# codelaboratoryltd/bng

Measured on AMD Instinct MI355X. Metric: mpps, higher is better.
Workload: dtype uint8; 1 GPU; model=bng-uplink-pipeline (dhcp_fastpath+antispoof+nat44+qos), benchmark=Mpps + p50 DHCP OFFER latency, 64B mix, 1M-sub table at 1/2/4/8 MI355X, global_batch=1048576, seq_len=512, svc_cus=0, parallelism=shard1-rss-dhcp-alltoall, n_subscribers=1000000

## Files before the change

bng_amd/dataplane/csrc/bng_device.h:

```cpp
#ifndef BNG_DEVICE_H
#define BNG_DEVICE_H

#include <hip/hip_runtime.h>
#include "bng_abi.h"

#define BNG_DEV __device__ __forceinline__

BNG_DEV uint64_t bng_mix64(uint64_t x) {
  x += 0x9E3779B97F4A7C15ULL;
  uint64_t z = x;
  z = (z ^ (z >> 30)) * 0xBF58476D1CE4E5B9ULL;
  z = (z ^ (z >> 27)) * 0x94D049BB133111EBULL;
  return z ^ (z >> 31);
}

BNG_DEV uint64_t bng_fnv1a64(const uint8_t* p, int n) {
  uint64_t h = 0xCBF29CE484222325ULL;
  for (int i = 0; i < n; ++i) { h ^= p[i]; h *= 0x100000001B3ULL; }
  return h;
}

BNG_DEV uint64_t bng_tuple_sig(uint32_t src_ip, uint32_t dst_ip,
                               uint16_t src_port, uint16_t dst_port,
                               uint8_t proto) {
  uint64_t a = ((uint64_t)src_ip << 32) | dst_ip;
  uint64_t b = ((uint64_t)src_port << 24) | ((uint64_t)dst_port << 8) | proto;
  uint64_t s = bng_mix64(bng_mix64(a) ^ b);
  s |= 1ULL;
  if (s == BNG_KEY_TOMBSTONE) s -= 2;
  return s;
}

BNG_DEV uint64_t bng_eim_sig(uint32_t ip, uint16_t port, uint8_t proto) {
  uint64_t s = bng_mix64(((uint64_t)ip << 24) | ((uint64_t)port << 8) | proto);
  s |= 1ULL;
  if (s == BNG_KEY_TOMBSTONE) s -= 2;
  return s;
}

BNG_DEV uint8_t  ld_u8 (const uint8_t* p)  { return *p; }
BNG_DEV uint16_t ld_u16be(const uint8_t* p) {
  return ((uint16_t)p[0] << 8) | p[1];
}
BNG_DEV uint32_t ld_u32be(const uint8_t* p) {
  return ((uint32_t)p[0] << 24) | ((uint32_t)p[1] << 16) |
         ((uint32_t)p[2] << 8) | p[3];
}
BNG_DEV void st_u16be(uint8_t* p, uint16_t v) {
  p[0] = (uint8_t)(v >> 8); p[1] = (uint8_t)v;
}
BNG_DEV void st_u32be(uint8_t* p, uint32_t v) {
  p[0] = (uint8_t)(v >> 24); p[1] = (uint8_t)(v >> 16);
  p[2] = (uint8_t)(v >> 8);  p[3] = (uint8_t)v;
}
BNG_DEV void bng_zero(uint8_t* p, int n) {
  int i = 0;
  while (((uintptr_t)(p + i) & 3) && i < n) p[i++] = 0;
  for (; i + 16 <= n && !((uintptr_t)(p + i) & 15); i += 16)
    *(uint4*)(p + i) = make_uint4(0, 0, 0, 0);
  for (; i + 4 <= n; i += 4) *(uint32_t*)(p + i) = 0;
  while (i < n) p[i++] = 0;
}

BNG_DEV void stat_inc(unsigned long long* counter, bool cond) {
  uint64_t mask = __ballot(cond);
  if (mask == 0) return;
  int leader = __ffsll((unsigned long long)mask) - 1;
  int lane = threadIdx.x & 63;
  if (lane == leader)
    atomicAdd(counter, (unsigned long long)__popcll(mask));
}

BNG_DEV uint32_t wave_count(bool cond) {
  return (uint32_t)__popcll((unsigned long long)__ballot(cond));
}

BNG_DEV uint32_t wave_sum32(uint32_t v) {
  for (int off = 32; off > 0; off >>= 1)
    v += __shfl_down(v, off, 64);
  return (uint32_t)__builtin_amdgcn_readfirstlane((int)v);
}

BNG_DEV void sb_zero(unsigned long long* sb, int n) {
  if ((int)threadIdx.x < n) sb[threadIdx.x] = 0;
  __syncthreads();
}

BNG_DEV void sb_fold(unsigned long long* sb, int slot, uint64_t cnt) {
  if (cnt && (threadIdx.x & 63) == 0)
    atomicAdd(&sb[slot], (unsigned long long)cnt);
}

BNG_DEV void sb_commit(const unsigned long long* sb, int base, int n,
                       unsigned long long* counters) {
  int k = (int)threadIdx.x - base;
  if (k >= 0 && k < n) {
    unsigned long long v = sb[base + k];
    if (v) atomicAdd(&counters[k], v);
  }
}

BNG_DEV void bng_publish_ready(uint8_t* ready_flag) {
  __builtin_amdgcn_fence(__ATOMIC_RELEASE, "agent");
  asm volatile("s_waitcnt vmcnt(0)" ::: "memory");
  __hip_atomic_store(ready_flag, (uint8_t)1, __ATOMIC_RELAXED,
                     __HIP_MEMORY_SCOPE_AGENT);
}

BNG_DEV bool bng_wait_ready(const uint8_t* ready_flag, int max_spins) {
  for (int i = 0; i < max_spins; ++i) {
    if (__hip_atomic_load(ready_flag, __ATOMIC_RELAXED,
                          __HIP_MEMORY_SCOPE_AGENT)) {
      __builtin_amdgcn_fence(__ATOMIC_ACQUIRE, "agent");
      return true;
    }
    __builtin_amdgcn_s_sleep(1);
  }
  return false;
}

BNG_DEV uint32_t ring_claim(bng_ring_header* hdr) {
  return atomicAdd(&hdr->widx, 1u);
}

#endif
```

bng_amd/dataplane/csrc/bng_kernels.hip:

```cpp
#include <hip/hip_runtime.h>
#include "bng_abi.h"
#include "bng_params.h"
#include "bng_device.h"
#include "bng_launch.h"


typedef __attribute__((address_space(1))) uint64_t gu64_t;

BNG_DEV uint64_t rlx_load64(const void* ptr) {
  return __hip_atomic_load((const uint64_t*)ptr, __ATOMIC_RELAXED,
                           __HIP_MEMORY_SCOPE_AGENT);
}
BNG_DEV void rlx_store64(void* ptr, uint64_t v) {
  __hip_atomic_store((uint64_t*)ptr, v, __ATOMIC_RELAXED,
                     __HIP_MEMORY_SCOPE_AGENT);
}

#ifndef BNG_SC1_PROBES
#define BNG_SC1_PROBES 1
#endif
BNG_DEV uint4 ld_probe16(const void* p) {
#if BNG_SC1_PROBES
  const uint64_t* q = (const uint64_t*)p;
  uint64_t a = rlx_load64(q), b = rlx_load64(q + 1);
// ... 113 lines not shown
  return &t[(slot + my_pos) & mask];
}

template <typename E>
BNG_DEV E* sig_find_or_claim(E* t, uint32_t mask, uint64_t sig,
                             bool* claimed, bool* found) {
  *claimed = false; *found = false;
  uint32_t slot = (uint32_t)sig & mask;
  for (int i = 0; i < BNG_MAX_PROBE; ++i) {
    E* e = &t[(slot + i) & mask];
    uint64_t k = __hip_atomic_load(&e->sig, __ATOMIC_RELAXED,
                                   __HIP_MEMORY_SCOPE_AGENT);
    if (k == sig) { *found = true; return e; }
    if (k == BNG_KEY_EMPTY) break;
  }
  for (int attempt = 0; attempt < 4; ++attempt) {
    int first_tomb = -1, first_tomb_pos = -1;
    for (int i = 0; i < BNG_MAX_PROBE; ++i) {
      E* e = &t[(slot + i) & mask];
      uint64_t k = __hip_atomic_load(&e->sig, __ATOMIC_RELAXED,
                                     __HIP_MEMORY_SCOPE_AGENT);
      if (k == sig) { *found = true; return e; }
      if (k == BNG_KEY_TOMBSTONE) {
        if (first_tomb < 0) {
          first_tomb = (int)((slot + i) & mask);
          first_tomb_pos = i;
        }
        continue;
      }
      if (k == BNG_KEY_EMPTY) {
        E* d = first_tomb >= 0 ? &t[first_tomb] : e;
        int d_pos = first_tomb >= 0 ? first_tomb_pos : i;
        uint64_t want = first_tomb >= 0 ? BNG_KEY_TOMBSTONE
                                        : BNG_KEY_EMPTY;
        if (__hip_atomic_compare_exchange_strong(
                &d->sig, &want, sig, __ATOMIC_RELAXED, __ATOMIC_RELAXED,
                __HIP_MEMORY_SCOPE_AGENT)) {
          return claim_dedup(t, mask, sig, slot, d_pos, claimed, found);
        }
        if (want == sig) { *found = true; return d; }
        if (first_tomb >= 0) { first_tomb = -1; first_tomb_pos = -1; --i; }
        continue;
      }
    }
    if (first_tomb < 0)
      return nullptr;
    E* d = &t[first_tomb];
    uint64_t want = BNG_KEY_TOMBSTONE;
    if (__hip_atomic_compare_exchange_strong(
            &d->sig, &want, sig, __ATOMIC_RELAXED, __ATOMIC_RELAXED,
            __HIP_MEMORY_SCOPE_AGENT)) {
      return claim_dedup(t, mask, sig, slot, first_tomb_pos, claimed,
                         found);
    }
    if (want == sig) { *found = true; return d; }
  }
  return nullptr;
}

template <typename E>
BNG_DEV E* sig_lookup(E* t, uint32_t mask, uint64_t sig) {
  uint32_t slot = (uint32_t)sig & mask;
  for (int i = 0; i < BNG_MAX_PROBE; ++i) {
    E* e = &t[(slot + i) & mask];
    uint64_t k = __hip_atomic_load(&e->sig, __ATOMIC_RELAXED,
                                   __HIP_MEMORY_SCOPE_AGENT);
    if (k == sig) return e;
    if (k == BNG_KEY_EMPTY) return nullptr;
  }
  return nullptr;
}

template <auto K, typename E>
BNG_DEV E* key_upsert_slot(E* t, uint32_t mask, uint64_t key) {
  uint32_t slot = (uint32_t)bng_mix64(key) & mask;
  E* tomb = nullptr;
  for (int i = 0; i < BNG_MAX_PROBE; ++i) {
    E* e = &t[(slot + i) & mask];
    uint64_t cur = rlx_load64(&(e->*K));
    if (cur == key) return e;
    if (cur == BNG_KEY_TOMBSTONE && !tomb) tomb = e;
    if (cur == BNG_KEY_EMPTY) {
      E* d = tomb ? tomb : e;
      uint64_t expect = tomb ? BNG_KEY_TOMBSTONE : BNG_KEY_EMPTY;
      if (__hip_atomic_compare_exchange_strong(
              &(d->*K), &expect, key, __ATOMIC_RELAXED, __ATOMIC_RELAXED,
              __HIP_MEMORY_SCOPE_AGENT))
        return d;
      tomb = nullptr;
    }
  }
  return nullptr;
}

template <auto K, typename E>
BNG_DEV E* key_find(E* t, uint32_t mask, uint64_t key) {
  uint32_t slot = (uint32_t)bng_mix64(key) & mask;
  for (int i = 0; i < BNG_MAX_PROBE; ++i) {
    E* e = &t[(slot + i) & mask];
    uint64_t cur = rlx_load64(&(e->*K));
    if (cur == key) return e;
    if (cur == BNG_KEY_EMPTY) return nullptr;
  }
  return nullptr;
}

template <typename E>
BNG_DEV E* ipkey_upsert_slot(E* t, uint32_t mask, uint32_t ip,
                             bool claim_if_absent, bool* full) {
  *full = false;
  uint32_t slot = (uint32_t)bng_mix64(ip) & mask;
  for (int i = 0; i < BNG_MAX_PROBE; ++i) {
    E* e = &t[(slot + i) & mask];
    uint32_t cur = __hip_atomic_load(&e->key_ip, __ATOMIC_RELAXED,
                                     __HIP_MEMORY_SCOPE_AGENT);
    if (cur == ip) return e;
    if (cur == 0) {
      if (!claim_if_absent) return nullptr;
      if (__hip_atomic_compare_exchange_strong(
              &e->key_ip, &cur, ip, __ATOMIC_RELAXED, __ATOMIC_RELAXED,
              __HIP_MEMORY_SCOPE_AGENT))
        return e;
    }
  }
  *full = true;
  return nullptr;
}

BNG_DEV bool tuple_eq(const bng_nat_tuple& a, const bng_nat_tuple& b) {
  return a.src_ip == b.src_ip && a.dst_ip == b.dst_ip &&
         a.src_port == b.src_port && a.dst_port == b.dst_port &&
         a.protocol == b.protocol;
}


struct pktctx {
  uint8_t* p;
  int len;
  int ip_off;
  int l4_off;
  uint8_t proto;
  uint32_t saddr, daddr;
  uint16_t sport, dport;
  uint16_t icmp_id;
  uint8_t tcp_flags;
  int vlan_offset;
  uint16_t s_tag, c_tag;
  bool tagged;
  bool l4_ok;
  uint32_t W[12];
  bool regs;
};

#define RG_B(c, o) (((c).W[(o) >> 2] >> (24 - 8 * ((o) & 3))) & 0xFFu)
BNG_DEV uint16_t rg_ld16(const pktctx& c, int o) {
  return (uint16_t)((RG_B(c, o) << 8) | RG_B(c, o + 1));
}
BNG_DEV void rg_st8(pktctx& c, int o, uint32_t v) {
  int i = o >> 2, sh = 24 - 8 * (o & 3);
  c.W[i] = (c.W[i] & ~(0xFFu << sh)) | ((v & 0xFFu) << sh);
}
BNG_DEV void rg_st16(pktctx& c, int o, uint32_t v) {
  rg_st8(c, o, v >> 8); rg_st8(c, o + 1, v);
}
BNG_DEV void rg_st32(pktctx& c, int o, uint32_t v) {
  rg_st16(c, o, v >> 16); rg_st16(c, o + 2, v);
}
BNG_DEV void rg_flush16_47(pktctx& c) {
  uint4* q = (uint4*)c.p;
  q[1] = make_uint4(__builtin_bswap32(c.W[4]), __builtin_bswap32(c.W[5]),
                    __builtin_bswap32(c.W[6]), __builtin_bswap32(c.W[7]));
  q[2] = make_uint4(__builtin_bswap32(c.W[8]), __builtin_bswap32(c.W[9]),
                    __builtin_bswap32(c.W[10]),
                    __builtin_bswap32(c.W[11]));
}

BNG_DEV bool parse_pkt_fast(pktctx& c, uint8_t* p, int len) {
  if (len < 48 || ((uintptr_t)p & 15)) return false;
  #pragma unroll
  for (int i = 0; i < 3; ++i) {
    uint4 v = ((const uint4*)p)[i];
    c.W[i * 4 + 0] = __builtin_bswap32(v.x);
    c.W[i * 4 + 1] = __builtin_bswap32(v.y);
    c.W[i * 4 + 2] = __builtin_bswap32(v.z);
    c.W[i * 4 + 3] = __builtin_bswap32(v.w);
  }
  #define BNG_B(o) ((c.W[(o) >> 2] >> (24 - 8 * ((o) & 3))) & 0xFFu)
  #define BNG_H(o) ((BNG_B(o) << 8) | BNG_B((o) + 1))
  uint32_t ethertype = BNG_H(12);
  if (ethertype != 0x0800) return false;
  if (BNG_B(14) != 0x45) return false;
  c.p = p; c.len = len; c.vlan_offset = 0; c.s_tag = c.c_tag = 0;
  c.tagged = false; c.l4_ok = false;
  c.regs = true;
  c.ip_off = 14;
  c.proto = (uint8_t)BNG_B(23);
  c.saddr = (BNG_H(26) << 16) | BNG_H(28);
  c.daddr = (BNG_H(30) << 16) | BNG_H(32);
  c.l4_off = 34;
  if (c.proto == 6 && len >= 54) {
    c.sport = (uint16_t)BNG_H(34);
    c.dport = (uint16_t)BNG_H(36);
    c.tcp_flags = (uint8_t)BNG_B(47);
    c.l4_ok = true;
  } else if (c.proto == 17 && len >= 42) {
    c.sport = (uint16_t)BNG_H(34);
    c.dport = (uint16_t)BNG_H(36);
    c.l4_ok = true;
  } else if (c.proto == 1 && len >= 42) {
    c.icmp_id = (uint16_t)BNG_H(38);
    c.l4_ok = true;
  }
  #undef BNG_B
  #undef BNG_H
  return true;
}

BNG_DEV bool parse_pkt_slow(pktctx& c, uint8_t* p, int len, bool want_vlan) {
  c.p = p; c.len = len; c.ip_off = -1; c.vlan_offset = 0;
  c.s_tag = c.c_tag = 0; c.tagged = false; c.l4_ok = false;
  c.regs = false;
  if (len < 14) return false;
  uint16_t proto = ld_u16be(p + 12);
  int off = 14;
  if (want_vlan && (proto == 0x8100 || proto == 0x88A8)) {
    if (len < off + 4) return false;
    c.tagged = true;
    c.s_tag = ld_u16be(p + off) & 0xFFF;
    proto = ld_u16be(p + off + 2);
    off += 4; c.vlan_offset = 4;
    if (proto == 0x8100) {
      if (len < off + 4) return false;
      c.c_tag = ld_u16be(p + off) & 0xFFF;
      proto = ld_u16be(p + off + 2);
      off += 4; c.vlan_offset = 8;
    }
  }
  if (proto != 0x0800 || len < off + 20) return false;
  c.ip_off = off;
  c.proto = p[off + 9];
  c.saddr = ld_u32be(p + off + 12);
  c.daddr = ld_u32be(p + off + 16);
  int ihl = (p[off] & 0xF) * 4;
  c.l4_off = off + ihl;
  if (c.proto == 6 && len >= c.l4_off + 20) {
    c.sport = ld_u16be(p + c.l4_off);
    c.dport = ld_u16be(p + c.l4_off + 2);
    c.tcp_flags = p[c.l4_off + 13];
    c.l4_ok = true;
  } else if (c.proto == 17 && len >= c.l4_off + 8) {
    c.sport = ld_u16be(p + c.l4_off);
    c.dport = ld_u16be(p + c.l4_off + 2);
    c.l4_ok = true;
  } else if (c.proto == 1 && len >= c.l4_off + 8) {
    c.icmp_id = ld_u16be(p + c.l4_off + 4);
    c.l4_ok = true;
  }
  return true;
}

BNG_DEV bool parse_pkt(pktctx& c, uint8_t* p, int len, bool want_vlan) {
  if (parse_pkt_fast(c, p, len)) return true;
  return parse_pkt_slow(c, p, len, want_vlan);
}


struct dhcp_tables {
  const bng_sub_entry* subs; uint32_t sub_mask;
  const bng_ip_pool* pools;  uint32_t n_pools;
  const bng_server_config* cfg;
  unsigned long long* stats;
  uint64_t now_sec;
};

struct dhcp_flags {
  bool vlan, total, hit, miss, expired, error, o82, bcast, ucast;
  BNG_DEV void clear() {
    vlan = total = hit = miss = expired = error = o82 = bcast = ucast = false;
  }
};

BNG_DEV void scan_dhcp_options(const uint8_t* p, int opt_off, int end,
                               uint8_t* msg_type, const uint8_t** cid,
                               int* cid_len) {
  *msg_type = 0; *cid = nullptr; *cid_len = 0;
  int i = opt_off;
  int limit = min(end, opt_off + 312);
  for (int iters = 0; iters < 64 && i < limit; ++iters) {
    uint8_t code = p[i];
    if (code == 0) { ++i; continue; }
    if (code == 255) break;
    if (i + 1 >= limit) break;
    uint8_t ln = p[i + 1];
    if (i + 2 + ln > limit) break;
    if (code == 53 && ln == 1) *msg_type = p[i + 2];
    else if (code == 82) {
      int j = i + 2, sub_end = i + 2 + ln;
      while (j + 2 <= sub_end) {
        uint8_t sc = p[j], sl = p[j + 1];
        if (j + 2 + sl > sub_end) break;
        if (sc == 1 && sl > 0 && sl <= 32) { *cid = p + j + 2; *cid_len = sl; }
        j += 2 + sl;
      }
    }
    i += 2 + ln;
  }
}

BNG_DEV int dhcp_process(uint8_t* p, int len, int stride,
                         const dhcp_tables& T, dhcp_flags& F,
                         uint16_t* out_len) {
  *out_len = (uint16_t)len;
  pktctx c;
  if (!parse_pkt(c, p, len, true)) {
    if (c.tagged) F.vlan = true;
    return BNG_PASS;
  }
  if (c.tagged) F.vlan = true;
  if (c.ip_off < 0 || c.proto != 17 || !c.l4_ok) return BNG_PASS;
  if (c.dport != 67) return BNG_PASS;
  int dhcp_off = c.l4_off + 8;
  if (len < dhcp_off + 240) return BNG_PASS;
  if (p[dhcp_off] != 1) return BNG_PASS;
  if (ld_u32be(p + dhcp_off + 236) != 0x63825363u) return BNG_PASS;

  F.total = true;

  uint8_t msg_type; const uint8_t* cid; int cid_len;
  scan_dhcp_options(p, dhcp_off + 240, len, &msg_type, &cid, &cid_len);
  if (msg_type != 1 && msg_type != 3) { F.miss = true; return BNG_PASS; }

  const bng_sub_entry* sub = nullptr;
  if (c.tagged) {
    uint64_t vk = BNG_KEY_VLAN | ((uint64_t)c.s_tag << 16) | c.c_tag;
    sub = sub_lookup(T.subs, T.sub_mask, vk);
  }
  if (!sub && cid) {
    uint8_t padded[32];
    #pragma unroll
    for (int i = 0; i < 32; ++i) padded[i] = (i < cid_len) ? cid[i] : 0;
    uint64_t ck = BNG_KEY_CIRCUIT | (bng_fnv1a64(padded, 32) >> 2);
    sub = sub_lookup(T.subs, T.sub_mask, ck);
    if (sub) F.o82 = true;
  }
  if (!sub) {
    uint64_t mac = 0;
    #pragma unroll
    for (int i = 0; i < 6; ++i) mac = (mac << 8) | p[dhcp_off + 28 + i];
    sub = sub_lookup(T.subs, T.sub_mask, mac);
  }
  if (!sub) { F.miss = true; return BNG_PASS; }
  if (T.now_sec > sub->lease_expiry) { F.expired = true; return BNG_PASS; }
  if (sub->pool_id >= T.n_pools) { F.error = true; return BNG_PASS; }
  const bng_ip_pool pool = T.pools[sub->pool_id];
  if (!pool.valid) { F.error = true; return BNG_PASS; }
  F.hit = true;

  const bng_server_config cfg = *T.cfg;
  uint8_t reply_type = (msg_type == 1) ? 2 : 5;
  uint32_t giaddr = ld_u32be(p + dhcp_off + 24);
  uint32_t server_ip = cfg.server_ip ? cfg.server_ip : pool.gateway;

  int ip_off = c.ip_off, udp_off = c.l4_off;
  if (giaddr != 0) {
    #pragma unroll
    for (int i = 0; i < 6; ++i) p[i] = p[6 + i];
    #pragma unroll
    for (int i = 0; i < 6; ++i) p[6 + i] = cfg.server_mac[i];
    st_u32be(p + ip_off + 12, server_ip);
    st_u32be(p + ip_off + 16, giaddr);
    st_u16be(p + udp_off, 67); st_u16be(p + udp_off + 2, 67);
    F.ucast = true;
  } else {
    uint16_t flags = ld_u16be(p + dhcp_off + 10);
    uint32_t ciaddr = ld_u32be(p + dhcp_off + 12);
    bool use_bcast = (flags & 0x8000) || ciaddr == 0;
    if (use_bcast) {
      #pragma unroll
      for (int i = 0; i < 6; ++i) p[i] = 0xFF;
      F.bcast = true;
    } else {
      #pragma unroll
      for (int i = 0; i < 6; ++i) p[i] = p[dhcp_off + 28 + i];
      F.ucast = true;
    }
    #pragma unroll
    for (int i = 0; i < 6; ++i) p[6 + i] = cfg.server_mac[i];
    st_u32be(p + ip_off + 12, server_ip);
    st_u32be(p + ip_off + 16, 0xFFFFFFFFu);
    st_u16be(p + udp_off, 67); st_u16be(p + udp_off + 2, 68);
  }
  p[ip_off + 8] = 64;
  st_u16be(p + udp_off + 6, 0);

  p[dhcp_off] = 2;
  p[dhcp_off + 3] = 0;
  st_u32be(p + dhcp_off + 16, sub->allocated_ip);
  st_u32be(p + dhcp_off + 20, server_ip);
  bng_zero(p + dhcp_off + 44, 192);

  uint8_t* o = p + dhcp_off + 240;
  int w = 0;
  o[w++] = 53; o[w++] = 1; o[w++] = reply_type;
  o[w++] = 54; o[w++] = 4; st_u32be(o + w, server_ip); w += 4;
  o[w++] = 51; o[w++] = 4; st_u32be(o + w, pool.lease_time); w += 4;
  uint32_t mask32 = (pool.prefix_len == 0) ? 0
      : (pool.prefix_len >= 32) ? 0xFFFFFFFFu
      : (0xFFFFFFFFu << (32 - pool.prefix_len));
  o[w++] = 1;  o[w++] = 4; st_u32be(o + w, mask32); w += 4;
  o[w++] = 3;  o[w++] = 4; st_u32be(o + w, pool.gateway); w += 4;
  if (pool.dns_primary) {
    uint8_t dl = pool.dns_secondary ? 8 : 4;
    o[w++] = 6; o[w++] = dl;
    st_u32be(o + w, pool.dns_primary); w += 4;
    if (pool.dns_secondary) { st_u32be(o + w, pool.dns_secondary); w += 4; }
  }
  o[w++] = 58; o[w++] = 4; st_u32be(o + w, pool.lease_time / 2); w += 4;
  o[w++] = 59; o[w++] = 4; st_u32be(o + w, (pool.lease_time * 7) / 8); w += 4;
  o[w++] = 255;

  int dhcp_len = 240 + w;
  int udp_len = 8 + dhcp_len;
  int ip_len = 20 + udp_len;
  int total = 14 + c.vlan_offset + ip_len;
  st_u16be(p + ip_off + 2, (uint16_t)ip_len);
  st_u16be(p + udp_off + 4, (uint16_t)udp_len);
  st_u16be(p + ip_off + 10, 0);
  uint32_t s = 0;
  #pragma unroll
  for (int i = 0; i < 10; ++i) s += ld_u16be(p + ip_off + 2 * i);
  s = (s & 0xFFFF) + (s >> 16); s = (s & 0xFFFF) + (s >> 16);
  st_u16be(p + ip_off + 10, (uint16_t)~s);

  *out_len = (uint16_t)min(total, stride);
  return BNG_TX;
}

enum {
  SB_DHCP = 0,
  SB_NAT = SB_DHCP + BNG_DHCP_NSTATS,
  SB_AS = SB_NAT + BNG_NAT_NSTATS,
  SB_QOS = SB_AS + BNG_AS_NSTATS,
  SB_N = SB_QOS + BNG_QOS_NSTATS
};

BNG_DEV void dhcp_count_stats(const dhcp_flags& F, unsigned long long* sb) {
  sb_fold(sb, SB_DHCP + BNG_ST_VLAN_PACKETS, wave_count(F.vlan));
  sb_fold(sb, SB_DHCP + BNG_ST_TOTAL_REQUESTS, wave_count(F.total));
  sb_fold(sb, SB_DHCP + BNG_ST_FASTPATH_HITS, wave_count(F.hit));
  sb_fold(sb, SB_DHCP + BNG_ST_FASTPATH_MISSES, wave_count(F.miss));
  sb_fold(sb, SB_DHCP + BNG_ST_CACHE_EXPIRED, wave_count(F.expired));
  sb_fold(sb, SB_DHCP + BNG_ST_ERRORS, wave_count(F.error));
  sb_fold(sb, SB_DHCP + BNG_ST_OPTION82_PRESENT, wave_count(F.o82));
  sb_fold(sb, SB_DHCP + BNG_ST_BROADCAST_REPLIES, wave_count(F.bcast));
  sb_fold(sb, SB_DHCP + BNG_ST_UNICAST_REPLIES, wave_count(F.ucast));
}

BNG_DEV void dhcp_commit_stats(const dhcp_flags& F, unsigned long long* st) {
  stat_inc(&st[BNG_ST_VLAN_PACKETS], F.vlan);
  stat_inc(&st[BNG_ST_TOTAL_REQUESTS], F.total);
  stat_inc(&st[BNG_ST_FASTPATH_HITS], F.hit);
  stat_inc(&st[BNG_ST_FASTPATH_MISSES], F.miss);
  stat_inc(&st[BNG_ST_CACHE_EXPIRED], F.expired);
  stat_inc(&st[BNG_ST_ERRORS], F.error);
  stat_inc(&st[BNG_ST_OPTION82_PRESENT], F.o82);
  stat_inc(&st[BNG_ST_BROADCAST_REPLIES], F.bcast);
  stat_inc(&st[BNG_ST_UNICAST_REPLIES], F.ucast);
}

__global__ void dhcp_fastpath_kernel(
    uint8_t* __restrict__ data, const uint16_t* __restrict__ in_len,
    uint16_t* __restrict__ out_len, uint8_t* __restrict__ verdict,
    int n, int stride,
    const bng_sub_entry* __restrict__ subs, uint32_t sub_mask,
    const bng_ip_pool* __restrict__ pools, uint32_t n_pools,
    const bng_server_config* __restrict__ cfg,
    unsigned long long* __restrict__ stats, uint64_t now_sec,
    const uint64_t* __restrict__ now_ptr) {
  if (now_ptr) now_sec = now_ptr[1];
  dhcp_tables T{subs, sub_mask, pools, n_pools, cfg, stats, now_sec};
  __shared__ unsigned long long sb[SB_N];
  sb_zero(sb, SB_N);
  int tid = blockIdx.x * blockDim.x + threadIdx.x;
  int nthreads = gridDim.x * blockDim.x;
  for (int base = 0; base < n; base += nthreads) {
    int pid = base + tid;
    dhcp_flags F; F.clear();
    if (pid < n) {
      uint16_t ol = in_len[pid];
      int v = dhcp_process(data + (size_t)pid * stride, in_len[pid], stride,
                           T, F, &ol);
      verdict[pid] = (uint8_t)v;
      out_len[pid] = ol;
    }
    dhcp_count_stats(F, sb);
  }
  __syncthreads();
  sb_commit(sb, SB_DHCP, BNG_DHCP_NSTATS, stats);
}

__global__ void __launch_bounds__(256, 1) dhcp_service_kernel(
    bng_svc_ctrl* __restrict__ ctrl,
    uint8_t* __restrict__ req,
    const uint16_t* __restrict__ in_len,
    uint16_t* __restrict__ out_len,
    uint8_t* __restrict__ verdict,
    uint8_t* __restrict__ scratch,
    int n_slots,
    uint32_t* __restrict__ ctrs,
    const bng_sub_entry* __restrict__ subs, uint32_t sub_mask,
    const bng_ip_pool* __restrict__ pools, uint32_t n_pools,
    const bng_server_config* __restrict__ cfg,
    unsigned long long* __restrict__ stats) {
  __shared__ uint32_t s_head, s_run, s_n;
  __shared__ uint64_t s_now;
  const int tid = threadIdx.x;
  const int nb = (int)gridDim.x, blk = (int)blockIdx.x;
  uint32_t done = __hip_atomic_load(&ctrl->tail, __ATOMIC_RELAXED,
                                    __HIP_MEMORY_SCOPE_SYSTEM);
  const int stride = (int)ctrl->stride;
  uint64_t idle = 0;
  const uint64_t idle_max = (uint64_t)ctrl->idle_exit_k * 1024u;
  uint64_t batches = 0;
  unsigned long long* served64 = (unsigned long long*)(ctrs + 4);
  for (;;) {
    if (tid == 0) {
      s_head = __hip_atomic_load(&ctrl->head, __ATOMIC_ACQUIRE,
                                 __HIP_MEMORY_SCOPE_SYSTEM);
      s_run = __hip_atomic_load(&ctrl->run, __ATOMIC_RELAXED,
                                __HIP_MEMORY_SCOPE_SYSTEM);
      s_n = ctrl->n_pkts;
      s_now = ctrl->now_sec;
    }
    __syncthreads();
    bool work = (s_head != done);
    if (!s_run || (!work && idle >= idle_max)) break;
    if (!work) {
      ++idle;
      __builtin_amdgcn_s_sleep(8);
      __syncthreads();
      continue;
    }
    idle = 0;
    int n = (int)s_n;
    if (n > n_slots) n = n_slots;
    const int lo = (int)((long)n * blk / nb);
    const int hi = (int)((long)n * (blk + 1) / nb);
    const size_t w0 = (size_t)lo * stride / 16;
    const int words = (hi - lo) * stride / 16;
    const uint4* src = (const uint4*)req + w0;
    uint4* dst = (uint4*)scratch + w0;
    for (int i = tid; i < words; i += blockDim.x) dst[i] = src[i];
    __syncthreads();
    dhcp_tables T{subs, sub_mask, pools, n_pools, cfg, stats, s_now};
    for (int pid = lo + tid; pid < hi; pid += blockDim.x) {
      dhcp_flags F; F.clear();
      uint16_t ol = in_len[pid];
      int v = dhcp_process(scratch + (size_t)pid * stride, in_len[pid],
                           stride, T, F, &ol);
      verdict[pid] = (uint8_t)v;
      out_len[pid] = ol;
      dhcp_commit_stats(F, stats);
    }
    __syncthreads();
    for (int i = tid; i < words; i += blockDim.x)
      ((uint4*)req)[w0 + i] = dst[i];
    __syncthreads();
    ++done; ++batches;
    if (tid == 0) {
      atomicAdd(served64, (unsigned long long)(hi - lo));
      uint32_t prev = __hip_atomic_fetch_add(&ctrs[0], 1u,
                                             __ATOMIC_ACQ_REL,
                                             __HIP_MEMORY_SCOPE_AGENT);
      if ((int)(prev % (uint32_t)nb) == nb - 1) {
        ctrl->served = *served64;
        ctrl->batches = batches;
        __hip_atomic_store(&ctrl->tail, done, __ATOMIC_RELEASE,
                           __HIP_MEMORY_SCOPE_SYSTEM);
      }
    }
    __syncthreads();
  }
  if (tid == 0) {
    uint32_t prev = __hip_atomic_fetch_add(&ctrs[1], 1u, __ATOMIC_ACQ_REL,
                                           __HIP_MEMORY_SCOPE_AGENT);
    if ((int)prev == nb - 1) {
      ctrl->served = *served64;
      __hip_atomic_store(&ctrl->exited, 1u, __ATOMIC_RELEASE,
// ... 564 lines not shown
    uint8_t* __restrict__ data, const uint16_t* __restrict__ in_len,
    uint8_t* __restrict__ verdict, int n, int stride, int is_egress,
    void* table, uint32_t mask,
    unsigned long long* stats, uint64_t now_ns) {
  __shared__ unsigned long long sb[SB_N];
  sb_zero(sb, SB_N);
  int tid = blockIdx.x * blockDim.x + threadIdx.x;
  int nthreads = gridDim.x * blockDim.x;
  for (int base = 0; base < n; base += nthreads) {
    int pid = base + tid;
    qos_flags F{false, false, 0};
    if (pid < n) {
      pktctx c;
      parse_pkt(c, data + (size_t)pid * stride, in_len[pid], false);
      int v;
      if (is_egress) {
        v = qos_process(c, (bng_qos_bucket*)table, mask, true, now_ns, F);
      } else {
        bng_subctx* e = (c.ip_off >= 0)
            ? subctx_lookup((bng_subctx*)table, mask, c.saddr) : nullptr;
        v = qos_process_ctx(c, e, now_ns, F);
      }
      verdict[pid] = (uint8_t)v;
    }
    qos_count_stats(F, sb);
  }
  __syncthreads();
  sb_commit(sb, SB_QOS, BNG_QOS_NSTATS, stats);
}


struct as_flags { bool allowed, dropped, logged, v4viol, v6viol; };

BNG_DEV void as_count_stats(const as_flags& F, unsigned long long* sb) {
  sb_fold(sb, SB_AS + BNG_AS_ALLOWED, wave_count(F.allowed));
  sb_fold(sb, SB_AS + BNG_AS_DROPPED, wave_count(F.dropped));
  sb_fold(sb, SB_AS + BNG_AS_LOGGED, wave_count(F.logged));
  sb_fold(sb, SB_AS + BNG_AS_V4_VIOLATIONS, wave_count(F.v4viol));
  sb_fold(sb, SB_AS + BNG_AS_V6_VIOLATIONS, wave_count(F.v6viol));
}

BNG_DEV void spoof_log_push(bng_spoof_event* ring, bng_ring_header* hdr,
                            const uint8_t* mac, uint8_t proto,
                            uint32_t spoofed, uint32_t allowed,
                            uint64_t now_ns) {
  if (!ring) return;
  uint32_t idx = ring_claim(hdr);
  bng_spoof_event* e = &ring[idx & ((1u << BNG_SPOOF_RING_LOG2) - 1)];
  e->timestamp = now_ns;
  #pragma unroll
  for (int i = 0; i < 6; ++i) e->src_mac[i] = mac[i];
  e->protocol = proto;
  e->spoofed_ip = spoofed; e->allowed_ip = allowed;
  #pragma unroll
  for (int i = 0; i < 16; ++i) { e->spoofed_ipv6[i] = 0; e->allowed_ipv6[i] = 0; }
}

BNG_DEV int antispoof_process_with(uint8_t* p, int len,
                              const bng_binding_entry* b,
                              const bng_antispoof_config* cfg,
                              bng_spoof_event* ring, bng_ring_header* hdr,
                              uint64_t now_ns, as_flags& F) {
  uint8_t mode = b ? b->mode : cfg->default_mode;
  if (mode == BNG_AS_DISABLED) { F.allowed = true; return BNG_FWD; }
  uint16_t proto = ld_u16be(p + 12);
  if (proto == 0x0800) {
    if (len < 34) return BNG_FWD;
    uint32_t src_ip = ld_u32be(p + 14 + 12);
    bool allowed = false;
    uint32_t bound_ip = 0;
    if (b && b->ipv4_valid) {
      bound_ip = b->ipv4_addr;
      if (mode == BNG_AS_STRICT || mode == BNG_AS_LOG_ONLY)
        allowed = (src_ip == bound_ip);
    } else if (mode == BNG_AS_LOOSE) {
      allowed = ip_in_intervals(cfg->allowed_lo, cfg->allowed_hi,
                                cfg->n_allowed_ranges, src_ip);
    }
    if (!allowed) {
      if (cfg->log_violations) {
        spoof_log_push(ring, hdr, p + 6, 4, src_ip, bound_ip, now_ns);
        F.logged = true;
      }
      if (mode == BNG_AS_LOG_ONLY) { F.allowed = true; return BNG_FWD; }
      F.dropped = true; F.v4viol = true;
      return BNG_DROP;
    }
    F.allowed = true; return BNG_FWD;
  }
  if (proto == 0x86DD) {
    if (len < 14 + 40) return BNG_FWD;
    bool allowed = false;
    if (b && b->ipv6_valid) {
      allowed = true;
      #pragma unroll
      for (int i = 0; i < 16; ++i)
        if (p[14 + 8 + i] != b->ipv6_addr[i]) { allowed = false; break; }
    } else if (mode == BNG_AS_LOOSE) {
      allowed = true;
    }
    if (!allowed && mode != BNG_AS_LOG_ONLY) {
      if (cfg->log_violations) {
        spoof_log_push(ring, hdr, p + 6, 6, 0, 0, now_ns);
        F.logged = true;
      }
      F.dropped = true; F.v6viol = true;
      return BNG_DROP;
    }
    F.allowed = true; return BNG_FWD;
  }
  F.allowed = true;
  return BNG_FWD;
}

BNG_DEV int antispoof_process(uint8_t* p, int len,
                              const bng_binding_entry* bindings,
                              uint32_t bmask,
                              const bng_antispoof_config* cfg,
                              bng_spoof_event* ring, bng_ring_header* hdr,
                              uint64_t now_ns, as_flags& F) {
  if (len < 14) return BNG_FWD;
  uint64_t mac = 0;
  #pragma unroll
  for (int i = 0; i < 6; ++i) mac = (mac << 8) | p[6 + i];
  const bng_binding_entry* b = binding_lookup(bindings, bmask, mac);
  return antispoof_process_with(p, len, b, cfg, ring, hdr, now_ns, F);
}

__global__ void antispoof_kernel(
    uint8_t* __restrict__ data, const uint16_t* __restrict__ in_len,
    uint8_t* __restrict__ verdict, int n, int stride,
    const bng_binding_entry* bindings, uint32_t bmask,
    const bng_antispoof_config* cfg,
    unsigned long long* stats,
    bng_spoof_event* ring, bng_ring_header* hdr, uint64_t now_ns) {
  __shared__ unsigned long long sb[SB_N];
  sb_zero(sb, SB_N);
  int tid = blockIdx.x * blockDim.x + threadIdx.x;
  int nthreads = gridDim.x * blockDim.x;
  for (int base = 0; base < n; base += nthreads) {
    int pid = base + tid;
    as_flags F{false, false, false, false, false};
    if (pid < n) {
      verdict[pid] = (uint8_t)antispoof_process(
          data + (size_t)pid * stride, in_len[pid], bindings, bmask, cfg,
          ring, hdr, now_ns, F);
    }
    as_count_stats(F, sb);
  }
  __syncthreads();
  sb_commit(sb, SB_AS, BNG_AS_NSTATS, stats);
}

__global__ __launch_bounds__(256, 5)
void uplink_pipeline_kernel(bng_uplink_params P) {
  if (P.now_ptr) { P.now_ns = P.now_ptr[0]; P.now_sec = P.now_ptr[1]; }
  dhcp_tables DT{P.subs, P.sub_mask, P.pools, P.n_pools, P.scfg,
                 P.dhcp_stats, P.now_sec};
  nat_tables NT{P.sessions, P.sess_mask, P.reverse, P.rev_mask, P.eim,
                P.eim_mask, P.subctx, P.subctx_mask, P.ncfg, P.hairpin_ips,
                P.n_hairpin, P.nat_stats, P.log_ring, P.log_hdr, P.now_ns};
  __shared__ unsigned long long sb[SB_N];
  sb_zero(sb, SB_N);
  int tid = blockIdx.x * blockDim.x + threadIdx.x;
  int nthreads = gridDim.x * blockDim.x;
  for (int base = 0; base < P.n; base += nthreads) {
    int i = base + tid;
    dhcp_flags DF; DF.clear();
    nat_flags NF; NF.clear();
    as_flags AF{false, false, false, false, false};
    qos_flags QF{false, false, 0};
    if (i < P.n) do {
      int pid = P.order ? P.order[i] : i;
      if ((unsigned)pid >= (unsigned)P.n) break;
      uint8_t* p = P.data + (size_t)pid * P.stride;
      int len = P.in_len[pid];
      uint16_t ol = (uint16_t)len;
      int v;
      pktctx c;
      uint16_t et = len >= 14 ? (uint16_t)((p[12] << 8) | p[13]) : 0;
      if (et == 0x8863 || et == 0x8864 || et == 0x0806) {
        P.verdict[pid] = (uint8_t)BNG_PASS;
        P.out_len[pid] = ol;
        break;
      }
      bool ip_ok = parse_pkt(c, p, len, true);
      bool is_dhcp = ip_ok && c.ip_off >= 0 && c.proto == 17 && c.l4_ok &&
                     c.dport == 67;
      if (is_dhcp) {
        v = dhcp_process(p, len, P.stride, DT, DF, &ol);
      } else if (ip_ok && !c.tagged && len >= 14) {
        uint64_t mac;
        if (c.regs) {
          mac = ((uint64_t)rg_ld16(c, 6) << 32) |
                ((uint64_t)rg_ld16(c, 8) << 16) | rg_ld16(c, 10);
        } else {
          mac = 0;
          #pragma unroll
          for (int j = 0; j < 6; ++j) mac = (mac << 8) | p[6 + j];
        }
        uint32_t s0 = (uint32_t)bng_mix64(mac) & P.bmask;
        uint32_t s1 = (uint32_t)bng_mix64(c.saddr) & P.subctx_mask;
        uint4 f0 = ld_probe16(&P.bindings[s0]);
        uint4 f1 = ld_probe16(&P.subctx[s1]);
        const bng_binding_entry* b =
            binding_lookup_hint(P.bindings, P.bmask, mac, s0, f0);
        v = antispoof_process_with(p, len, b, P.acfg, P.spoof_ring,
                                   P.spoof_hdr, P.now_ns, AF);
        if (v == BNG_FWD) {
          bng_subctx* ctxe = subctx_lookup_hint(
              P.subctx, P.subctx_mask, c.saddr, s1, f1);
          v = nat_egress_process(c, NT, NF, ctxe, true);
          if (v == BNG_FWD)
            v = qos_process_ctx(c, ctxe, P.now_ns, QF);
        }
      } else {
        v = antispoof_process(p, len, P.bindings, P.bmask, P.acfg,
                              P.spoof_ring, P.spoof_hdr, P.now_ns, AF);
        if (v == BNG_FWD && ip_ok && !c.tagged) {
          bng_subctx* ctxe = subctx_lookup(P.subctx, P.subctx_mask, c.saddr);
          v = nat_egress_process(c, NT, NF, ctxe, true);
          if (v == BNG_FWD)
            v = qos_process_ctx(c, ctxe, P.now_ns, QF);
        }
      }
      P.verdict[pid] = (uint8_t)v;
      P.out_len[pid] = ol;
    } while (0);
    dhcp_count_stats(DF, sb);
    nat_count_stats(NF, sb);
    as_count_stats(AF, sb);
    qos_count_stats(QF, sb);
  }
  __syncthreads();
  sb_commit(sb, SB_DHCP, BNG_DHCP_NSTATS, P.dhcp_stats);
  sb_commit(sb, SB_NAT, BNG_NAT_NSTATS, P.nat_stats);
  sb_commit(sb, SB_AS, BNG_AS_NSTATS, P.as_stats);
  sb_commit(sb, SB_QOS, BNG_QOS_NSTATS, P.qos_stats);
}

__global__ __launch_bounds__(256, 5)
void downlink_pipeline_kernel(bng_uplink_params P) {
  if (P.now_ptr) { P.now_ns = P.now_ptr[0]; P.now_sec = P.now_ptr[1]; }
  nat_tables NT{P.sessions, P.sess_mask, P.reverse, P.rev_mask, P.eim,
                P.eim_mask, P.subctx, P.subctx_mask, P.ncfg, P.hairpin_ips,
                P.n_hairpin, P.nat_stats, P.log_ring, P.log_hdr, P.now_ns};
  __shared__ unsigned long long sb[SB_N];
  sb_zero(sb, SB_N);
  int tid = blockIdx.x * blockDim.x + threadIdx.x;
  int nthreads = gridDim.x * blockDim.x;
  for (int base = 0; base < P.n; base += nthreads) {
    int i = base + tid;
    nat_flags NF; NF.clear();
    qos_flags QF{false, false, 0};
    if (i < P.n) {
      int pid = P.order ? P.order[i] : i;
      uint8_t* p = P.data + (size_t)pid * P.stride;
      int len = P.in_len[pid];
      pktctx c;
      bool ip_ok = parse_pkt(c, p, len, false);
      int v = BNG_FWD;
      if (ip_ok) {
        v = nat_ingress_process(c, NT, NF);
        if (v == BNG_FWD && c.ip_off >= 0) {
          c.daddr = ld_u32be(p + c.ip_off + 16);
          v = qos_process(c, P.qos_eg, P.qos_eg_mask, true,
                          P.now_ns, QF);
        }
      }
      P.verdict[pid] = (uint8_t)v;
      P.out_len[pid] = (uint16_t)len;
    }
    nat_count_stats(NF, sb);
    qos_count_stats(QF, sb);
  }
  __syncthreads();
  sb_commit(sb, SB_NAT, BNG_NAT_NSTATS, P.nat_stats);
  sb_commit(sb, SB_QOS, BNG_QOS_NSTATS, P.qos_stats);
}

__global__ void pkt_class_kernel(const uint8_t* __restrict__ data,
                                 const uint16_t* __restrict__ in_len,
                                 uint8_t* __restrict__ cls, int n,
                                 int stride) {
  int tid = blockIdx.x * blockDim.x + threadIdx.x;
  int nthreads = gridDim.x * blockDim.x;
  for (int pid = tid; pid < n; pid += nthreads) {
    pktctx c;
    bool ip_ok = parse_pkt(c, const_cast<uint8_t*>(data) +
                           (size_t)pid * stride, in_len[pid], true);
    cls[pid] = (ip_ok && c.ip_off >= 0 && c.proto == 17 && c.l4_ok &&
                c.dport == 67) ? 1 : 0;
  }
}


__global__ void sess_import_kernel(
    bng_nat_session* sess, uint32_t sess_mask,
    bng_nat_reverse* rev, uint32_t rev_mask,
    bng_eim_entry* eim, uint32_t eim_mask,
    const bng_sess_export* batch, int n, int* rc) {
  int i = blockIdx.x * blockDim.x + threadIdx.x;
  if (i >= n) return;
  bng_sess_export e = batch[i];
  uint64_t sig = bng_tuple_sig(e.src_ip, e.dst_ip, e.src_port, e.dst_port,
                               e.protocol);
  bool claimed, found;
  bng_nat_session* s = sig_find_or_claim(sess, sess_mask, sig,
                                         &claimed, &found);
  if (!s) { if (rc) rc[i] = 1; return; }
  s->key = bng_nat_tuple{e.src_ip, e.dst_ip, e.src_port, e.dst_port,
                         e.protocol, {0, 0, 0}};
  s->nat_ip = e.nat_ip; s->nat_port = e.nat_port;
  s->orig_port = e.src_port; s->orig_ip = e.src_ip;
  s->state = e.state; s->is_hairpin = e.is_hairpin;
  s->last_seen = e.last_seen; s->created = e.created;
  s->packets_out = 0; s->packets_in = 0;
  s->bytes_out = 0; s->bytes_in = 0;
  bng_publish_ready(&s->ready);

  uint64_t rsig = bng_tuple_sig(e.dst_ip, e.nat_ip, e.dst_port,
                                e.nat_port, e.protocol);
  bng_nat_reverse* r = sig_find_or_claim(rev, rev_mask, rsig,
                                         &claimed, &found);
  if (r) {
    r->key = bng_nat_tuple{e.dst_ip, e.nat_ip, e.dst_port, e.nat_port,
                           e.protocol, {0, 0, 0}};
    r->orig = s->key;
    bng_publish_ready(&r->ready);
  } else if (rc) {
    rc[i] = 2;
  }

  if (e.flags & 1) {
    uint64_t esig = bng_eim_sig(e.src_ip, e.src_port, e.protocol);
    bng_eim_entry* m = sig_find_or_claim(eim, eim_mask, esig,
                                         &claimed, &found);
    if (m) {
      m->internal_ip = e.src_ip; m->internal_port = e.src_port;
      m->protocol = e.protocol;
      m->external_ip = e.nat_ip; m->external_port = e.eim_port;
      m->created = e.created; m->last_used = e.last_seen;
      if (claimed) m->ref_count = 1;
// ... 618 lines not shown
```

Baseline: 1946 Mpps.

## Build DHCP replies in registers with wide 16-byte stores and reuse parsed context

Adds a wide DHCP reply path that loads the BOOTP header into registers, rewrites Ethernet/IP/UDP/BOOTP fields in register words, and writes the reply and options with 16-byte vector stores instead of byte-wise stores. The uplink kernel now passes its already-parsed packet context to DHCP processing rather than reparsing. The FNV hash over the circuit ID is computed inline without a padded stack buffer. Launch bounds occupancy hint drops from 5 to 2, allowing more registers but fewer resident waves. The wide path is only used when stride is at least 336 and register parsing succeeded, and it zero-fills the rest of the frame.

```diff
diff --git a/bng_amd/dataplane/csrc/bng_device.h b/bng_amd/dataplane/csrc/bng_device.h
--- a/bng_amd/dataplane/csrc/bng_device.h
+++ b/bng_amd/dataplane/csrc/bng_device.h
@@ -12,12 +12,6 @@
   z = (z ^ (z >> 30)) * 0xBF58476D1CE4E5B9ULL;
   z = (z ^ (z >> 27)) * 0x94D049BB133111EBULL;
   return z ^ (z >> 31);
-}
-
-BNG_DEV uint64_t bng_fnv1a64(const uint8_t* p, int n) {
-  uint64_t h = 0xCBF29CE484222325ULL;
-  for (int i = 0; i < n; ++i) { h ^= p[i]; h *= 0x100000001B3ULL; }
-  return h;
 }
 
 BNG_DEV uint64_t bng_tuple_sig(uint32_t src_ip, uint32_t dst_ip,
diff --git a/bng_amd/dataplane/csrc/bng_kernels.hip b/bng_amd/dataplane/csrc/bng_kernels.hip
--- a/bng_amd/dataplane/csrc/bng_kernels.hip
+++ b/bng_amd/dataplane/csrc/bng_kernels.hip
@@ -289,20 +289,38 @@
   bool regs;
 };
 
+template <int N> BNG_DEV uint32_t w_ld8(const uint32_t (&W)[N], int o) {
+  return (W[o >> 2] >> (24 - 8 * (o & 3))) & 0xFFu;
+}
+template <int N> BNG_DEV uint32_t w_ld16(const uint32_t (&W)[N], int o) {
+  return (w_ld8(W, o) << 8) | w_ld8(W, o + 1);
+}
+template <int N> BNG_DEV uint32_t w_ld32(const uint32_t (&W)[N], int o) {
+  return (w_ld16(W, o) << 16) | w_ld16(W, o + 2);
+}
+template <int N> BNG_DEV void w_st8(uint32_t (&W)[N], int o, uint32_t v) {
+  int i = o >> 2, sh = 24 - 8 * (o & 3);
+  W[i] = (W[i] & ~(0xFFu << sh)) | ((v & 0xFFu) << sh);
+}
+template <int N> BNG_DEV void w_st16(uint32_t (&W)[N], int o, uint32_t v) {
+  w_st8(W, o, v >> 8); w_st8(W, o + 1, v);
+}
+template <int N> BNG_DEV void w_st32(uint32_t (&W)[N], int o, uint32_t v) {
+  w_st16(W, o, v >> 16); w_st16(W, o + 2, v);
+}
+template <int N> BNG_DEV uint4 w_chunk(const uint32_t (&W)[N], int k) {
+  return make_uint4(__builtin_bswap32(W[4 * k]),
+                    __builtin_bswap32(W[4 * k + 1]),
+                    __builtin_bswap32(W[4 * k + 2]),
+                    __builtin_bswap32(W[4 * k + 3]));
+}
 #define RG_B(c, o) (((c).W[(o) >> 2] >> (24 - 8 * ((o) & 3))) & 0xFFu)
 BNG_DEV uint16_t rg_ld16(const pktctx& c, int o) {
   return (uint16_t)((RG_B(c, o) << 8) | RG_B(c, o + 1));
 }
-BNG_DEV void rg_st8(pktctx& c, int o, uint32_t v) {
-  int i = o >> 2, sh = 24 - 8 * (o & 3);
-  c.W[i] = (c.W[i] & ~(0xFFu << sh)) | ((v & 0xFFu) << sh);
-}
-BNG_DEV void rg_st16(pktctx& c, int o, uint32_t v) {
-  rg_st8(c, o, v >> 8); rg_st8(c, o + 1, v);
-}
-BNG_DEV void rg_st32(pktctx& c, int o, uint32_t v) {
-  rg_st16(c, o, v >> 16); rg_st16(c, o + 2, v);
-}
+BNG_DEV void rg_st8(pktctx& c, int o, uint32_t v) { w_st8(c.W, o, v); }
+BNG_DEV void rg_st16(pktctx& c, int o, uint32_t v) { w_st16(c.W, o, v); }
+BNG_DEV void rg_st32(pktctx& c, int o, uint32_t v) { w_st32(c.W, o, v); }
 BNG_DEV void rg_flush16_47(pktctx& c) {
   uint4* q = (uint4*)c.p;
   q[1] = make_uint4(__builtin_bswap32(c.W[4]), __builtin_bswap32(c.W[5]),
@@ -444,12 +462,127 @@
   }
 }
 
-BNG_DEV int dhcp_process(uint8_t* p, int len, int stride,
-                         const dhcp_tables& T, dhcp_flags& F,
-                         uint16_t* out_len) {
+enum {
+  BNG_DHCP_OPT_OFF = 282,
+  BNG_DHCP_MAX_OPTS = 50,
+  BNG_DHCP_WIDE_MIN_STRIDE = 336
+};
+
+struct dhcp_reply {
+  uint32_t yiaddr, server_ip;
+  uint8_t reply_type;
+};
+
+BNG_DEV uint32_t pool_netmask(const bng_ip_pool& pool) {
+  return (pool.prefix_len == 0) ? 0
+      : (pool.prefix_len >= 32) ? 0xFFFFFFFFu
+      : (0xFFFFFFFFu << (32 - pool.prefix_len));
+}
+
+template <int NDNS>
+BNG_DEV void dhcp_wide_options(uint8_t* p, const dhcp_reply& R,
+                               const bng_ip_pool& pool) {
+  uint32_t O[16];
+  #pragma unroll
+  for (int i = 0; i < 16; ++i) O[i] = 0;
+  int o = 6;
+  w_st32(O, o, 0x63825363u); o += 4;
+  w_st8(O, o, 53); w_st8(O, o + 1, 1); w_st8(O, o + 2, R.reply_type); o += 3;
+  w_st8(O, o, 54); w_st8(O, o + 1, 4); w_st32(O, o + 2, R.server_ip); o += 6;
+  w_st8(O, o, 51); w_st8(O, o + 1, 4); w_st32(O, o + 2, pool.lease_time);
+  o += 6;
+  w_st8(O, o, 1); w_st8(O, o + 1, 4); w_st32(O, o + 2, pool_netmask(pool));
+  o += 6;
+  w_st8(O, o, 3); w_st8(O, o + 1, 4); w_st32(O, o + 2, pool.gateway); o += 6;
+  if (NDNS) {
+    w_st8(O, o, 6); w_st8(O, o + 1, 4 * NDNS);
+    w_st32(O, o + 2, pool.dns_primary);
+    if (NDNS == 2) w_st32(O, o + 6, pool.dns_secondary);
+    o += 2 + 4 * NDNS;
+  }
+  w_st8(O, o, 58); w_st8(O, o + 1, 4); w_st32(O, o + 2, pool.lease_time / 2);
+  o += 6;
+  w_st8(O, o, 59); w_st8(O, o + 1, 4);
+  w_st32(O, o + 2, (pool.lease_time * 7) / 8); o += 6;
+  w_st8(O, o, 255); o += 1;
+  uint4* q = (uint4*)(p + 272);
+  q[0] = w_chunk(O, 0); q[1] = w_chunk(O, 1); q[2] = w_chunk(O, 2);
+  uint4 t = w_chunk(O, 3);
+  if (NDNS == 0) {
+    *(uint16_t*)(p + 320) = (uint16_t)t.x;
+  } else {
+    *(uint2*)(p + 320) = make_uint2(t.x, t.y);
+    if (NDNS == 2) *(uint32_t*)(p + 328) = t.z;
+  }
+}
+
+BNG_DEV int dhcp_reply_wide(pktctx& c, uint32_t (&X)[12],
+                            const dhcp_reply& R, const bng_ip_pool& pool,
+                            const bng_server_config& cfg, dhcp_flags& F) {
+  uint8_t* p = c.p;
+  const int ndns = pool.dns_primary ? (pool.dns_secondary ? 2 : 1) : 0;
+  const int w = 40 + (ndns ? 2 + 4 * ndns : 0);
+  uint32_t giaddr = w_ld32(X, 66 - 48);
+  uint32_t smac_hi = ((uint32_t)cfg.server_mac[0] << 8) | cfg.server_mac[1];
+  uint32_t smac_lo = ((uint32_t)cfg.server_mac[2] << 24) |
+                     ((uint32_t)cfg.server_mac[3] << 16) |
+                     ((uint32_t)cfg.server_mac[4] << 8) | cfg.server_mac[5];
+  uint32_t dst_ip, dport;
+  if (giaddr != 0) {
+    uint32_t hi = rg_ld16(c, 6);
+    uint32_t lo = ((uint32_t)rg_ld16(c, 8) << 16) | rg_ld16(c, 10);
+    rg_st16(c, 0, hi); rg_st32(c, 2, lo);
+    dst_ip = giaddr; dport = 67;
+    F.ucast = true;
+  } else {
+    uint32_t flags = w_ld16(X, 52 - 48), ciaddr = w_ld32(X, 54 - 48);
+    if ((flags & 0x8000) || ciaddr == 0) {
+      rg_st16(c, 0, 0xFFFFu); rg_st32(c, 2, 0xFFFFFFFFu);
+      F.bcast = true;
+    } else {
+      rg_st16(c, 0, w_ld16(X, 70 - 48)); rg_st32(c, 2, w_ld32(X, 72 - 48));
+      F.ucast = true;
+    }
+    dst_ip = 0xFFFFFFFFu; dport = 68;
+  }
+  rg_st16(c, 6, smac_hi); rg_st32(c, 8, smac_lo);
+  rg_st32(c, 26, R.server_ip); rg_st32(c, 30, dst_ip);
+  rg_st16(c, 34, 67); rg_st16(c, 36, dport);
+  rg_st8(c, 22, 64);
+  rg_st16(c, 40, 0);
+  rg_st8(c, 42, 2);
+  rg_st8(c, 45, 0);
+  rg_st16(c, 16, 20 + 8 + 240 + w);
+  rg_st16(c, 38, 8 + 240 + w);
+  rg_st16(c, 24, 0);
+  uint32_t s = 0;
+  #pragma unroll
+  for (int i = 0; i < 10; ++i) s += rg_ld16(c, 14 + 2 * i);
+  s = (s & 0xFFFF) + (s >> 16); s = (s & 0xFFFF) + (s >> 16);
+  rg_st16(c, 24, ~s & 0xFFFFu);
+
+  w_st32(X, 58 - 48, R.yiaddr);
+  w_st32(X, 62 - 48, R.server_ip);
+  w_st16(X, 86 - 48, 0); X[10] = 0; X[11] = 0;
+
+  uint4* q = (uint4*)p;
+  q[0] = w_chunk(c.W, 0); q[1] = w_chunk(c.W, 1); q[2] = w_chunk(c.W, 2);
+  q[3] = w_chunk(X, 0); q[4] = w_chunk(X, 1); q[5] = w_chunk(X, 2);
+  #pragma unroll
+  for (int i = 6; i < 17; ++i) q[i] = make_uint4(0, 0, 0, 0);
+  if (ndns == 0) dhcp_wide_options<0>(p, R, pool);
+  else if (ndns == 1) dhcp_wide_options<1>(p, R, pool);
+  else dhcp_wide_options<2>(p, R, pool);
+  return BNG_DHCP_OPT_OFF + w;
+}
+
+BNG_DEV int dhcp_process_ctx(pktctx& c, bool parsed, int stride,
+                             const dhcp_tables& T, dhcp_flags& F,
+                             uint16_t* out_len) {
+  uint8_t* p = c.p;
+  const int len = c.len;
   *out_len = (uint16_t)len;
-  pktctx c;
-  if (!parse_pkt(c, p, len, true)) {
+  if (!parsed) {
     if (c.tagged) F.vlan = true;
     return BNG_PASS;
   }
@@ -458,8 +591,29 @@
   if (c.dport != 67) return BNG_PASS;
   int dhcp_off = c.l4_off + 8;
   if (len < dhcp_off + 240) return BNG_PASS;
-  if (p[dhcp_off] != 1) return BNG_PASS;
-  if (ld_u32be(p + dhcp_off + 236) != 0x63825363u) return BNG_PASS;
+  const bool wide = c.regs && stride >= BNG_DHCP_WIDE_MIN_STRIDE;
+  uint32_t X[12];
+  #pragma unroll
+  for (int i = 0; i < 12; ++i) X[i] = 0;
+  if (wide) {
+    if (RG_B(c, 42) != 1) return BNG_PASS;
+    const uint4* q = (const uint4*)p;
+    uint4 m = q[17];
+    uint32_t cookie = (__builtin_bswap32(m.y) << 16) |
+                      (__builtin_bswap32(m.z) >> 16);
+    if (cookie != 0x63825363u) return BNG_PASS;
+    #pragma unroll
+    for (int i = 0; i < 3; ++i) {
+      uint4 v = q[3 + i];
+      X[i * 4 + 0] = __builtin_bswap32(v.x);
+      X[i * 4 + 1] = __builtin_bswap32(v.y);
+      X[i * 4 + 2] = __builtin_bswap32(v.z);
+      X[i * 4 + 3] = __builtin_bswap32(v.w);
+    }
+  } else {
+    if (p[dhcp_off] != 1) return BNG_PASS;
+    if (ld_u32be(p + dhcp_off + 236) != 0x63825363u) return BNG_PASS;
+  }
 
   F.total = true;
 
@@ -473,17 +627,23 @@
     sub = sub_lookup(T.subs, T.sub_mask, vk);
   }
   if (!sub && cid) {
-    uint8_t padded[32];
-    #pragma unroll
-    for (int i = 0; i < 32; ++i) padded[i] = (i < cid_len) ? cid[i] : 0;
-    uint64_t ck = BNG_KEY_CIRCUIT | (bng_fnv1a64(padded, 32) >> 2);
+    uint64_t h = 0xCBF29CE484222325ULL;
+    for (int i = 0; i < 32; ++i) {
+      h ^= (i < cid_len) ? cid[i] : 0;
+      h *= 0x100000001B3ULL;
+    }
+    uint64_t ck = BNG_KEY_CIRCUIT | (h >> 2);
     sub = sub_lookup(T.subs, T.sub_mask, ck);
     if (sub) F.o82 = true;
   }
   if (!sub) {
     uint64_t mac = 0;
-    #pragma unroll
-    for (int i = 0; i < 6; ++i) mac = (mac << 8) | p[dhcp_off + 28 + i];
+    if (wide) {
+      mac = ((uint64_t)w_ld16(X, 70 - 48) << 32) | w_ld32(X, 72 - 48);
+    } else {
+      #pragma unroll
+      for (int i = 0; i < 6; ++i) mac = (mac << 8) | p[dhcp_off + 28 + i];
+    }
     sub = sub_lookup(T.subs, T.sub_mask, mac);
   }
   if (!sub) { F.miss = true; return BNG_PASS; }
@@ -495,8 +655,14 @@
 
   const bng_server_config cfg = *T.cfg;
   uint8_t reply_type = (msg_type == 1) ? 2 : 5;
+  uint32_t server_ip = cfg.server_ip ? cfg.server_ip : pool.gateway;
+  if (wide) {
+    dhcp_reply R{sub->allocated_ip, server_ip, reply_type};
+    int total = dhcp_reply_wide(c, X, R, pool, cfg, F);
+    *out_len = (uint16_t)min(total, stride);
+    return BNG_TX;
+  }
   uint32_t giaddr = ld_u32be(p + dhcp_off + 24);
-  uint32_t server_ip = cfg.server_ip ? cfg.server_ip : pool.gateway;
 
   int ip_off = c.ip_off, udp_off = c.l4_off;
   if (giaddr != 0) {
@@ -541,10 +707,7 @@
   o[w++] = 53; o[w++] = 1; o[w++] = reply_type;
   o[w++] = 54; o[w++] = 4; st_u32be(o + w, server_ip); w += 4;
   o[w++] = 51; o[w++] = 4; st_u32be(o + w, pool.lease_time); w += 4;
-  uint32_t mask32 = (pool.prefix_len == 0) ? 0
-      : (pool.prefix_len >= 32) ? 0xFFFFFFFFu
-      : (0xFFFFFFFFu << (32 - pool.prefix_len));
-  o[w++] = 1;  o[w++] = 4; st_u32be(o + w, mask32); w += 4;
+  o[w++] = 1;  o[w++] = 4; st_u32be(o + w, pool_netmask(pool)); w += 4;
   o[w++] = 3;  o[w++] = 4; st_u32be(o + w, pool.gateway); w += 4;
   if (pool.dns_primary) {
     uint8_t dl = pool.dns_secondary ? 8 : 4;
@@ -571,6 +734,14 @@
 
   *out_len = (uint16_t)min(total, stride);
   return BNG_TX;
+}
+
+BNG_DEV int dhcp_process(uint8_t* p, int len, int stride,
+                         const dhcp_tables& T, dhcp_flags& F,
+                         uint16_t* out_len) {
+  pktctx c;
+  bool parsed = parse_pkt(c, p, len, true);
+  return dhcp_process_ctx(c, parsed, stride, T, F, out_len);
 }
 
 enum {
@@ -1441,7 +1612,7 @@
   sb_commit(sb, SB_AS, BNG_AS_NSTATS, stats);
 }
 
-__global__ __launch_bounds__(256, 5)
+__global__ __launch_bounds__(256, 2)
 void uplink_pipeline_kernel(bng_uplink_params P) {
   if (P.now_ptr) { P.now_ns = P.now_ptr[0]; P.now_sec = P.now_ptr[1]; }
   dhcp_tables DT{P.subs, P.sub_mask, P.pools, P.n_pools, P.scfg,
@@ -1477,7 +1648,7 @@
       bool is_dhcp = ip_ok && c.ip_off >= 0 && c.proto == 17 && c.l4_ok &&
                      c.dport == 67;
       if (is_dhcp) {
-        v = dhcp_process(p, len, P.stride, DT, DF, &ol);
+        v = dhcp_process_ctx(c, true, P.stride, DT, DF, &ol);
       } else if (ip_ok && !c.tagged && len >= 14) {
         uint64_t mac;
         if (c.regs) {
```

Measured after the change: 2073 Mpps, median of 6. +6.5%, better.
